# swesterfeld/audiowmark

Hardware: AMD Instinct MI355X
Metric: audio seconds watermarked+decoded per wall-second (xRT), 44.1 kHz stereo (higher is better)
Workload: dtype f32; 1 GPU; 60 min stereo 44.1 kHz white noise per GPU resident in HBM, add+get incl. payload decode, payload 0123456789abcdef0011223344556677, strength 10; parallelism=1 GPU, patterns=108, payload_matches=104, ranks_seen=1

## Files before the change

### audiowmark_amd/binding.py

```python
import ctypes as C
import os

import numpy as np

_HERE = os.path.dirname(os.path.abspath(__file__))
N_BANDS = 81
BLOCK_FRAMES = 2226
SOFT_BITS = 858


class AwmError(RuntimeError):
    pass


def library_path():
    return os.path.join(_HERE, "libawm_hip.so")




def _load_hip_runtime():
    candidates = []
    try:
        import torch
# ... 114 lines not shown
lib.awm_add_watermark_batch_keys_d.argtypes = [_vp, _vp, C.c_char_p, C.c_size_t, _vp, _vp, _vp, C.c_int]
lib.awm_get_watermark_batch_keys_d.argtypes = [_vp, _vp, C.c_size_t, _vp, _vp, C.c_int, C.c_int, C.c_size_t, _vp, _vp]
lib.awm_decode_chunk_d.argtypes = [_vp, _vp, _vp, C.c_size_t, C.c_int, C.c_int, C.c_size_t, _vp]
lib.awm_tab_up_down.argtypes = [_vp, C.c_int, C.c_int, _vp, _vp]
lib.awm_tab_bit_pos.argtypes = [_vp, _vp]
lib.awm_tab_mix_entries.argtypes = [_vp, _vp]
lib.awm_tab_bit_order.argtypes = [_vp, C.c_size_t, _vp]
lib.awm_tab_frame_mod.argtypes = [_vp, C.c_char_p, _vp]
lib.awm_tab_frame_mod_template.argtypes = [_vp, _vp]
lib.awm_tab_sync_bits.argtypes = [_vp, C.c_int, _vp]
lib.awm_tab_window.argtypes = [C.c_size_t, _vp]
lib.awm_tab_synth_window.argtypes = [_vp]
lib.awm_conv_encode.argtypes = [C.c_int, _vp, C.c_size_t, _vp]
lib.awm_test_gen_noise.argtypes = [_vp, C.c_size_t, _vp]


class RawFormat(C.Structure):
    _fields_ = [("n_channels", C.c_int), ("sample_rate", C.c_int), ("bit_depth", C.c_int), ("encoding", C.c_int), ("big_endian", C.c_int)]


lib.awm_add_watermark_file.argtypes = [_vp, _vp, C.c_char_p, C.c_char_p, C.c_char_p, C.POINTER(RawFormat), C.POINTER(RawFormat)]
lib.awm_add_stream_watermark_file.argtypes = [_vp, _vp, C.c_char_p, C.c_char_p, C.c_char_p, C.POINTER(RawFormat), C.POINTER(RawFormat), C.c_size_t]
lib.awm_add_stream_create_at.argtypes = [_vp, _vp, C.c_char_p, C.c_int, C.c_size_t, C.c_size_t, C.POINTER(_vp)]
lib.awm_debug_sync_db_sliding_d.argtypes = [_vp, _vp, C.c_size_t, C.c_int, _vp, C.c_size_t, C.c_int, C.c_int, _vp]
lib.awm_debug_sync_db_sliding_rows_d.argtypes = [_vp, _vp, C.c_size_t, C.c_int, _vp, _vp, C.c_size_t, C.c_int, C.c_int, _vp, _vp, C.c_longlong, C.c_longlong,
                                                 _vp, _vp, C.c_int, C.c_int, C.c_int, _vp, _vp, C.c_longlong, _vp, C.c_longlong]
lib.awm_get_watermark_file.argtypes = [_vp, _vp, C.c_char_p, C.POINTER(RawFormat), C.c_size_t, _vp]
lib.awm_add_get_watermark_file.argtypes = [_vp, _vp, C.c_char_p, C.c_char_p, C.c_char_p, C.POINTER(RawFormat), C.POINTER(RawFormat), C.c_size_t, _vp]
lib.awm_add_stream_create.argtypes = [_vp, _vp, C.c_char_p, C.c_int, C.c_size_t, C.POINTER(_vp)]
lib.awm_add_stream_destroy.argtypes = [_vp]
lib.awm_add_stream_destroy.restype = None
lib.awm_add_stream_input.argtypes = [_vp]
lib.awm_add_stream_input.restype = C.c_void_p
lib.awm_add_stream_push.argtypes = [_vp, C.c_size_t, C.c_int, _vp, _vp]
lib.awm_add_mix_payloads_d.argtypes = [_vp, _vp, _vp, C.c_size_t, C.c_size_t, C.c_int, _vp, C.c_double, C.c_size_t, _vp, _vp, _vp,
                                       C.c_size_t, C.c_size_t]
lib.awm_add_stream_create_payloads_at.argtypes = [_vp, _vp, _vp, C.c_size_t, C.c_int, C.c_size_t, C.c_size_t, C.POINTER(_vp)]
lib.awm_add_stream_payloads.argtypes = [_vp]
lib.awm_add_stream_payloads.restype = C.c_size_t
lib.awm_add_stream_push_payloads.argtypes = [_vp, C.c_size_t, C.c_int, _vp, _vp]
lib.awm_add_watermark_payloads_file.argtypes = [_vp, _vp, _vp, C.c_size_t, C.c_char_p, _vp, C.POINTER(RawFormat), C.POINTER(RawFormat)]
lib.awm_add_stream_watermark_payloads_file.argtypes = [_vp, _vp, _vp, C.c_size_t, C.c_char_p, _vp, C.POINTER(RawFormat), C.POINTER(RawFormat),
                                                       C.c_size_t]
lib.awm_debug_set_payloads_file_tile.argtypes = [C.c_int]
lib.awm_debug_set_payloads_file_tile.restype = None

# ... 520 lines not shown

    def add_watermark_payloads_file(self, key, payloads, in_path, out_paths, raw_in=None, raw_out=None, zero_frames=None):
        payloads = list(payloads)
        outs = check_payload_paths(payloads, in_path, out_paths)
        hexes = (C.c_char_p * len(payloads))(*[p.encode() for p in payloads])
        paths = (C.c_char_p * len(payloads))(*outs)
        rin = C.byref(raw_in) if raw_in is not None else None
        rout = C.byref(raw_out) if raw_out is not None else None
        if zero_frames is not None:
            _check(lib.awm_add_stream_watermark_payloads_file(self._h, key_bytes(key), hexes, len(payloads), os.fsencode(in_path), paths, rin, rout,
                                                              zero_frames), "awm_add_stream_watermark_payloads_file")
            return
        _check(lib.awm_add_watermark_payloads_file(self._h, key_bytes(key), hexes, len(payloads), os.fsencode(in_path), paths, rin, rout),
               "awm_add_watermark_payloads_file")

    def add_get_watermark_file(self, key, payload_hex, in_path, out_path, raw_in=None, raw_out=None):
        return self._patterns(lib.awm_add_get_watermark_file, "awm_add_get_watermark_file", self._h, key_bytes(key), payload_hex.encode(),
                              os.fsencode(in_path), os.fsencode(out_path), C.byref(raw_in) if raw_in is not None else None,
                              C.byref(raw_out) if raw_out is not None else None)

    def get_watermark_file(self, key, in_path, raw_in=None):
        return self._patterns(lib.awm_get_watermark_file, "awm_get_watermark_file", self._h, key_bytes(key), os.fsencode(in_path),
                              C.byref(raw_in) if raw_in is not None else None)

    def sync_db_sliding(self, pcm, bases, count, ld=72):
        import torch
        n, ch = _pcm_shape(pcm)
        b = torch.as_tensor(bases, dtype=torch.int64, device=pcm.device).contiguous()
        out = torch.zeros((b.numel(), 81, ld), dtype=torch.float32, device=pcm.device)
        _check(lib.awm_debug_sync_db_sliding_d(self._h, _dev_ptr(pcm), n, ch, C.c_void_p(b.data_ptr()), b.numel(), count, ld, _dev_ptr(out)),
               "awm_debug_sync_db_sliding_d")
        self.synchronize()
        return out

    def sync_db_sliding_rows(self, pcm, n_frames, bases, counts, count0, rows_per_plane, row_perm, band_pos, first, last, out, have,
                             tail=None, stream_range=None, range_index=None, range_div=1, tables_per_slice=0):
        import torch
        n, ch = _pcm_shape(pcm)
        assert 0 <= n_frames <= n
        want = ((bases, torch.int64, 1), (counts, torch.int32, 1), (row_perm, torch.int32, 0), (band_pos, torch.uint8, 0), (out, torch.float32, 3),
                (have, torch.int8, 2), (tail, torch.float32, 2), (stream_range, torch.int64, 2), (range_index, torch.int32, 1))
        for t, dtype, dim in want:
            assert t is None or (t.dtype == dtype and t.is_cuda and t.is_contiguous() and (not dim or t.dim() == dim))
        assert bases.numel() == counts.numel() and out.shape[1] == 60 and out.shape[0] == have.shape[0] and (tail is None or tail.shape[0] == out.shape[0])
        opt = lambda t: _dev_ptr(t) if t is not None else None
        _check(lib.awm_debug_sync_db_sliding_rows_d(self._h, _dev_ptr(pcm), n_frames, ch, _dev_ptr(bases), _dev_ptr(counts), bases.numel(), count0,
# ... 358 lines not shown
```

### audiowmark_amd/csrc/hip/kernels.hh

```
#pragma once
#include <hip/hip_runtime.h>
#include <cstddef>
#include <cstdint>

#if defined(__HIP_DEVICE_COMPILE__) && !defined(__gfx950__)
#error "audiowmark_amd's HIP kernels are written for gfx950 (MI355X) only"
#endif

namespace awmk {

struct DevTables
{
  const float2 *tw512;
  const float2 *tw1024;
  const float  *window;
  const float  *synth;
  const double2 *slide;
  const double2 *tw512d;
  const float2 *slide32;
};

hipError_t launch_stft_full (hipStream_t st, const DevTables& t, const float *pcm, int n_channels,
                             long long start_index, long long hop, long long frame_count, float2 *out);

struct AddMixArgs
{
  const float *pcm_in;
  float       *out;
  long long    n_frames;
  int          n_channels;
  const int8_t *frame_mod;
  float        neg_delta_up;
  float        neg_delta_down;
  long long    first_frame;
  const float *halo_before;
  const float *halo_after;
  unsigned int *block_max;
  long long    first_block;
  long long    n_blocks;
  int          limiter_block;
  int          frames_per_span;
  int          block_frames = 2226;
  int          frames_pad_start = 250;
// ... 361 lines not shown
```

### audiowmark_amd/csrc/hip/kernels.hip

```cpp
#include "kernels.hh"
#include "awm_fft.hip.h"
#include <cstdlib>
#include <algorithm>
#include <type_traits>

namespace awmk {

constexpr int NB = 81;
constexpr int MIN_BAND = 20;
constexpr int WAVES = 4;

typedef const int __attribute__ ((address_space (4))) *const_int_ptr;

__device__ __forceinline__ void
load_shared_tables (const DevTables& t, float2 *s_tw, float *s_win, float2 *s_twb)
{
  fft512_load_twiddles (t.tw512, s_tw);
  for (int i = threadIdx.x; i < 1024; i += blockDim.x)
    s_win[i] = t.window[i];
  if (s_twb)
    for (int i = threadIdx.x; i < NB; i += blockDim.x)
      s_twb[i] = t.tw1024[MIN_BAND + i];
}

// ... 51 lines not shown
        }
    }
  else
    {
#pragma unroll
      for (int j = 0; j < 8; j++)
        {
          const int x = 2 * (lane + 64 * j);
          v[2 * j]     = x < avail     ? p[(long long) x * C]       : 0.f;
          v[2 * j + 1] = x + 1 < avail ? p[(long long) (x + 1) * C] : 0.f;
        }
    }
}

__device__ __forceinline__ void
window_pack (const float (&v)[16], const float *s_win, int lane, float2 (&z)[8])
{
  const float2 *w2 = reinterpret_cast<const float2 *> (s_win);
#pragma unroll
  for (int j = 0; j < 8; j++)
    {
      const float2 w = lds_ld (&w2[lane + 64 * j]);
      z[j] = make_float2 (__fmul_rn (v[2 * j], w.x), __fmul_rn (v[2 * j + 1], w.y));
    }
}

__global__ void __launch_bounds__ (64 * WAVES)
stft_full_kernel (DevTables t, const float *pcm, int C, long long start_index, long long hop, long long frame_count, float2 *out)
{
  __shared__ float2 s_tw[512];
  __shared__ float  s_win[1024];
  __shared__ float2 s_x[WAVES][XBUF_ELEMS];
  load_shared_tables (t, s_tw, s_win, nullptr);
  __syncthreads();

  const int lane = threadIdx.x & 63, wave = threadIdx.x >> 6;
  const long long item = (long long) blockIdx.x * WAVES + wave;
  if (item >= frame_count * C)
    return;
  const long long f = item / C;
  const int ch = int (item % C);
  float2 *xbuf = s_x[wave];

  float v[16];
  fetch_channel (pcm, start_index + f * hop, 1024, C, ch, lane, v);
  float2 z[8];
// ... 469 lines not shown

  for (long long m = s - 1; m <= e; m++)
    {
      if (OPAQUE)
        {
          lane = lane0;
          asm volatile ("" : "+v" (lane));
        }
      int avail;
      const float *src = frame_source<true> (a.pcm_in, a.n_frames, C, F, m, a.halo_before, a.halo_after, avail);
      float in[CV][16];
      float2 d[CV][8];
      if (avail > 0)
        {
          if constexpr (CV == 2)
            fetch_stereo (src, 0, avail, lane, in[0], in[1]);
          else
            fetch_channel (src, 0, avail, C, ch0, lane, in[0]);
          const long long g = a.first_frame + m;
          const long long row = (frame_number0 + g) % total_rows;
          const int8_t *mod_row = a.frame_mod + row * NB;
          if constexpr (CV == 2 && PAIR)
            {
              window_pack (in[0], s_win, lane, d[0]);
              window_pack (in[1], s_win, lane, d[1]);
              frame_delta2 (d[0], d[1], mod_row, a.neg_delta_up, a.neg_delta_down, xbuf, zd, s_tw, s_tw3, s_twb, lane);
            }
          else
            {
#pragma unroll
              for (int c = 0; c < CV; c++)
                {
                  window_pack (in[c], s_win, lane, d[c]);
                  frame_delta (d[c], mod_row, a.neg_delta_up, a.neg_delta_down, xbuf, zd, s_tw, s_tw3, s_twb, lane);
                }
            }
        }
      else
        {
#pragma unroll
          for (int c = 0; c < CV; c++)
            {
#pragma unroll
              for (int j = 0; j < 16; j++)
                in[c][j] = 0.f;
#pragma unroll
              for (int j = 0; j < 8; j++)
                d[c][j] = make_float2 (0.f, 0.f);
// ... 138 lines not shown
          if constexpr (CV == 2)
            fetch_stereo (src, 0, avail, lane, in[0], in[1]);
          else
            fetch_channel (src, 0, avail, C, ch0, lane, in[0]);
          long long row = (frame_number0 + m) % total_rows;
          if constexpr (SPAN)
            row = (frame_number0 + sp.first_frame + m) % total_rows;
#pragma unroll
          for (int pass = 0; pass < 2; pass++)
            {
              const int k = MIN_BAND + lane + 64 * pass;
              mod[pass] = 0;
#pragma unroll
              for (int p = 0; p < PT; p++)
                if (p < a.n_out && k <= 100)
                  {
                    const int v = a.o[p].frame_mod[row * NB + (k - MIN_BAND)];
                    mod[pass] |= (v ? (v == 1 ? 3 : 1) : 0) << (2 * p);
                  }
            }
          const float e_up = __int_as_float (__builtin_amdgcn_readfirstlane (__float_as_int (0.5f * a.neg_delta_up)));
          const float e_down = __int_as_float (__builtin_amdgcn_readfirstlane (__float_as_int (0.5f * a.neg_delta_down)));
          float2 z[CV][8];
#pragma unroll
          for (int c = 0; c < CV; c++)
            window_pack (in[c], s_win, lane, z[c]);
          if constexpr (CV == 2)
            frame_forward2 (z[0], z[1], xbuf, s_tw, lane);
          else
            frame_forward (z[0], xbuf, s_tw, lane);
#pragma unroll
          for (int pass = 0; pass < 2; pass++)
            {
              const int k = MIN_BAND + lane + 64 * pass;
#pragma unroll
              for (int c = 0; c < CV; c++)
                d_up[c][pass] = d_down[c][pass] = zero;
              if (k <= 100)
                {
                  const float2 w = s_twb[k - MIN_BAND];
#pragma unroll
                  for (int c = 0; c < CV; c++)
                    {
                      float2 X;
                      if (CV == 2 && c == 1)
                        X = real_split (lds_ld (&xbuf[zposb (k)]), lds_ld (&xbuf[zposb (512 - k)]), w);
                      else if (CV == 2)
                        X = real_split (lds_ld (&xbuf[zpos (k)]), lds_ld (&xbuf[zpos (512 - k)]), w);
                      else
                        X = real_split (xbuf[zpos (k)], xbuf[zpos (512 - k)], w);
                      const float abs2 = X.x * X.x + X.y * X.y;
                      if (abs2 > 1e-14f)
                        {
// ... 861 lines not shown
  if (n_channels < 1 || seg.pre < 0 || seg.first_sample < seg.pre || (long long) limiter_block * n_channels < MIX_RUN)
    return hipErrorInvalidValue;
  hipLaunchKernelGGL (mix_max_segment_kernel, dim3 (unsigned ((n_values + MIX_RUN - 1) / MIX_RUN)), dim3 (256), 0, st, seg, n_channels, limiter_block);
  return hipGetLastError();
}

__global__ void
fill_u32_kernel (unsigned int *p, unsigned int v, size_t n)
{
  const size_t i = (size_t) blockIdx.x * blockDim.x + threadIdx.x;
  if (i < n)
    p[i] = v;
}
hipError_t
launch_fill_u32 (hipStream_t st, unsigned int *p, unsigned int v, size_t n)
{
  if (!n)
    return hipSuccess;
  hipLaunchKernelGGL (fill_u32_kernel, dim3 (unsigned ((n + 255) / 256)), dim3 (256), 0, st, p, v, n);
  return hipGetLastError();
}


__device__ __forceinline__ long long
sync_stream_base (const SyncDbArgs& a, long long stream)
{
  if (a.stream_base)
    return a.stream_base[stream];
  if (a.streams_per_slice > 0)
    return a.base0 + (stream % a.streams_per_slice) * a.base_stride + (stream / a.streams_per_slice) * a.slice_stride;
  return a.base0 + stream * a.base_stride;
}

__device__ __forceinline__ void
sync_stream_range (const SyncDbArgs& a, long long stream, long long& first, long long& last)
{
  first = a.first;
  last = a.last;
  if (a.stream_range)
    {
      const long long g = stream / a.range_div;
      const long long slice = a.range_index ? a.range_index[g] : g;
      first = a.stream_range[2 * slice];
      last = a.stream_range[2 * slice + 1];
      if (first < 0)
        first = last = 0x7fffffffffffffffLL;
    }
}


template<int CV, bool SPLIT, int TLD> __global__ void __launch_bounds__ (64 * WAVES)
sync_db_kernel (DevTables t, SyncDbArgs a)
{
  constexpr int TILE_LD = TLD, TILE_MAX = TLD - 1, SPLIT_COLS = TILE_MAX / 2;
  __shared__ float2 s_tw[512];
  __shared__ float  s_win[1024];
  __shared__ float2 s_twb[NB];
  __shared__ float2 s_x[WAVES][XBUF_ELEMS];
  __shared__ float  s_tile[NB * TILE_LD];
  __shared__ char   s_have[TILE_MAX];
  const int lane = threadIdx.x & 63, wave = threadIdx.x >> 6;
  if (a.silent_frames_are_zero && a.skip_unread_silent_tiles)
    {
      long long stream = blockIdx.y, tile_idx = blockIdx.x;
      if (a.xcd_interleave)
        {
          const long long j = blockIdx.x >> 3;
          stream = j % a.n_streams;
          tile_idx = (j / a.n_streams) * 8 + (blockIdx.x & 7);
        }
      const long long base = sync_stream_base (a, stream);
      const int count = a.stream_count ? a.stream_count[stream] : a.count0;
      long long sil_first, sil_last;
      sync_stream_range (a, stream, sil_first, sil_last);
      const long long tile0 = tile_idx * a.tile_frames;
      if (tile0 >= count)
        return;
      const long long n_here = (count - tile0) < a.tile_frames ? count - tile0 : a.tile_frames;
      const long long idx_before = base + (tile0 - 2) * a.hop, idx_after = base + (tile0 + n_here + 1) * a.hop;
      const int C = a.n_channels;
      if ((idx_after + 1024) * C < sil_first || idx_before * C > sil_last)
        return;
    }
  load_shared_tables (t, s_tw, s_win, s_twb);
  __syncthreads();

  long long stream = blockIdx.y, tile_idx = blockIdx.x;
  if (a.xcd_interleave)
    {
      const long long j = blockIdx.x >> 3;
      stream = j % a.n_streams;
      tile_idx = (j / a.n_streams) * 8 + (blockIdx.x & 7);
    }
  const int plane_ch = blockIdx.z;
  const long long base = sync_stream_base (a, stream);
  const int count = a.stream_count ? a.stream_count[stream] : a.count0;
  long long sil_first, sil_last;
  sync_stream_range (a, stream, sil_first, sil_last);
  const int TF = a.tile_frames;
  const long long tile0 = tile_idx * TF;
  if (tile0 >= count)
    return;
  const int C = a.n_channels;
  float2 *xbuf = s_x[wave];
  const int n_here = (count - tile0) < TF ? int (count - tile0) : TF;

  for (int ff = wave; ff < n_here; ff += WAVES)
    {
      const long long idx = base + (tile0 + ff) * a.hop;
      const long long f_first = idx * C, f_last = (idx + 1024) * C;
      const bool outside = idx < 0 || idx + 1024 > a.n_frames;
      const bool skip = (f_last < sil_first) || (f_first > sil_last) || outside;
      float acc0 = 0.f, acc1 = 0.f;
      float split0 = 0.f, split1 = 0.f;
      if (!skip)
        {
          if (CV == 2)
            {
              float in[2][16];
              fetch_stereo (a.pcm, idx, 1024, lane, in[0], in[1]);
              float2 za[8], zb[8];
              window_pack (in[0], s_win, lane, za);
              window_pack (in[1], s_win, lane, zb);
              fft512_forward2 (za, zb, xbuf, s_tw, lane);
              const int k0 = MIN_BAND + lane, k1 = MIN_BAND + 64 + lane;
              const bool second = lane < NB - 64;
              float2 pa[4], pb[4];
              lds_st (&xbuf[0 * 64 + lane], za[0]);
              lds_st (&xbuf[1 * 64 + lane], za[1]);
              lds_st (&xbuf[6 * 64 + lane], za[6]);
              lds_st (&xbuf[7 * 64 + lane], za[7]);
              wave_sync();
              pa[0] = lds_ld (&xbuf[zpos (k0)]);
              pa[1] = lds_ld (&xbuf[zpos (512 - k0)]);
              pa[2] = lds_ld (&xbuf[zpos (second ? k1 : k0)]);
              pa[3] = lds_ld (&xbuf[zpos (512 - (second ? k1 : k0))]);
              wave_sync();
              lds_st (&xbuf[0 * 64 + lane], zb[0]);
              lds_st (&xbuf[1 * 64 + lane], zb[1]);
              lds_st (&xbuf[6 * 64 + lane], zb[6]);
              lds_st (&xbuf[7 * 64 + lane], zb[7]);
              wave_sync();
              pb[0] = lds_ld (&xbuf[zpos (k0)]);
              pb[1] = lds_ld (&xbuf[zpos (512 - k0)]);
              pb[2] = lds_ld (&xbuf[zpos (second ? k1 : k0)]);
              pb[3] = lds_ld (&xbuf[zpos (512 - (second ? k1 : k0))]);
              wave_sync();
              const float2 w0 = s_twb[lane], w1 = s_twb[second ? 64 + lane : lane];
              acc0 = __fadd_rn (acc0, db_from_complex (real_split (pa[0], pa[1], w0)));
              if (second)
                acc1 = __fadd_rn (acc1, db_from_complex (real_split (pa[2], pa[3], w1)));
              if (SPLIT)
                {
                  split0 = acc0;
                  split1 = acc1;
                  acc0 = acc1 = 0.f;
                }
              acc0 = __fadd_rn (acc0, db_from_complex (real_split (pb[0], pb[1], w0)));
              if (second)
                acc1 = __fadd_rn (acc1, db_from_complex (real_split (pb[2], pb[3], w1)));
            }
          else
            {
              const int c_begin = a.per_channel ? plane_ch : 0, c_end = a.per_channel ? plane_ch + 1 : C;
              for (int c = c_begin; c < c_end; c++)
                {
                  float in[16];
                  fetch_channel (a.pcm, idx, 1024, C, c, lane, in);
                  float2 z[8];
// ... 60 lines not shown
          float *out = a.out + stream * a.out_stream_stride + (long long) p * NB * a.ld + tile0;
          for (int i = threadIdx.x; i < NB * n_here; i += blockDim.x)
            {
              const int band = i / n_here, ff = i - band * n_here;
              out[band * a.ld + ff] = s_tile[band * TILE_LD + p * SPLIT_COLS + ff];
            }
        }
    }
  else
    {
      const long long plane = a.per_channel ? plane_ch : 0;
      float *out = a.out + stream * a.out_stream_stride + plane * NB * a.ld + tile0;
      for (int i = threadIdx.x; i < NB * n_here; i += blockDim.x)
        {
          const int band = i / n_here, ff = i - band * n_here;
          out[band * a.ld + ff] = s_tile[band * TILE_LD + ff];
        }
    }
  if (a.have && plane_ch == 0)
    for (int i = threadIdx.x; i < n_here; i += blockDim.x)
      a.have[stream * a.have_stream_stride + tile0 + i] = s_have[i];
}

hipError_t
launch_sync_db (hipStream_t st, const DevTables& t, const SyncDbArgs& a)
{
  if (a.n_streams <= 0 || a.tile_frames <= 0 || a.tile_frames > 72)
    return a.n_streams <= 0 ? hipSuccess : hipErrorInvalidValue;
  int max_count = a.count0;
  if (max_count <= 0)
    return hipSuccess;
  const unsigned tiles = unsigned ((max_count + a.tile_frames - 1) / a.tile_frames);
  if (a.n_streams > 65535LL * 1)
    {
      SyncDbArgs b = a;
      long long done = 0;
      while (done < a.n_streams)
        {
          const long long n = (a.n_streams - done) > 65535 ? 65535 : (a.n_streams - done);
          b.n_streams = n;
          b.base0 = a.base0 + done * a.base_stride;
          b.stream_base = a.stream_base ? a.stream_base + done : nullptr;
          b.stream_count = a.stream_count ? a.stream_count + done : nullptr;
          b.out = a.out + done * a.out_stream_stride;
          b.have = a.have ? a.have + done * a.have_stream_stride : nullptr;
          hipError_t e = launch_sync_db (st, t, b);
          if (e != hipSuccess)
            return e;
          done += n;
        }
      return hipSuccess;
    }
  const bool small = a.tile_frames <= 32;
  if (a.n_channels == 2 && a.per_channel)
    {
      SyncDbArgs b = a;
      b.tile_frames = 16;
      const unsigned split_tiles = unsigned ((max_count + b.tile_frames - 1) / b.tile_frames);
      hipLaunchKernelGGL ((sync_db_kernel<2, true, 33>), dim3 (split_tiles, unsigned (a.n_streams), 1), dim3 (64 * WAVES), 0, st, t, b);
      return hipGetLastError();
    }
  const unsigned planes = a.per_channel ? unsigned (a.n_channels) : 1u;
  dim3 grid (tiles, unsigned (a.n_streams), planes);
  SyncDbArgs b = a;
  if (!a.stream_base && !a.stream_count && a.n_streams >= 2 && a.n_streams <= 8 && planes == 1)
    {
      b.xcd_interleave = 1;
      grid = dim3 (unsigned (((tiles + 7) / 8) * 8 * a.n_streams), 1, 1);
    }
  if (a.n_channels == 2 && !a.per_channel)
    {
      if (small)
        hipLaunchKernelGGL ((sync_db_kernel<2, false, 33>), grid, dim3 (64 * WAVES), 0, st, t, b);
      else
        hipLaunchKernelGGL ((sync_db_kernel<2, false, 73>), grid, dim3 (64 * WAVES), 0, st, t, b);
    }
  else
    {
      if (small)
        hipLaunchKernelGGL ((sync_db_kernel<1, false, 33>), grid, dim3 (64 * WAVES), 0, st, t, b);
      else
        hipLaunchKernelGGL ((sync_db_kernel<1, false, 73>), grid, dim3 (64 * WAVES), 0, st, t, b);
    }
  return hipGetLastError();
}

constexpr int SL_TILE = 16;

__device__ __forceinline__ double
dpp_from_lower_lane (double v)
{
  const int lo = __builtin_amdgcn_update_dpp (0, __double2loint (v), 0x138, 0xf, 0xf, true);
  const int hi = __builtin_amdgcn_update_dpp (0, __double2hiint (v), 0x138, 0xf, 0xf, true);
  return __hiloint2double (hi, lo);
}
// ... 1966 lines not shown
```

### audiowmark_amd/csrc/host/capi_kernels.cc

```cpp
#include "context.hh"
#include "syncfinder.hh"
#include "wmget.hh"
#include "wmspeed.hh"
#include "utils.hh"
#include "wmfile.hh"
#include <sys/stat.h>
#include <atomic>
#include <future>
#include <thread>
#include <tuple>
#include <algorithm>
#include <cmath>
#include <cstdlib>
#include <cstring>
#include <memory>

using namespace awm;
namespace awm { Key capi_key (const uint8_t key[16]); }
namespace awm { extern int g_key_tables_on_device; int clip_key_tables_check (awm_ctx *ctx, const uint8_t *keys, size_t n_keys, long long mismatch_out[9]); }

namespace {

constexpr int LIMITER_BLOCK = Params::mark_sample_rate * int (Params::limiter_block_size_ms) / 1000;
const float LIMITER_CEILING = float (Params::limiter_ceiling);
// ... 899 lines not shown
      const int zero = 0;
      AWM_HIP_CHECK (hipMemcpyAsync (ctx->ws_misc.ptr, &zero, sizeof (int), hipMemcpyHostToDevice, ctx->stream));
      AWM_HIP_CHECK (hipMemcpyAsync (ctx->ws_misc.as<char>() + sizeof (int), pos.data(), pos.size(), hipMemcpyHostToDevice, ctx->stream));
      da.row_perm = ctx->ws_misc.as<int>();
      da.band_pos = ctx->ws_misc.as<unsigned char>() + sizeof (int);
      da.rows_per_plane = 1;
      da.out_stream_stride = 60 * 64;
      if (awmk::sliding_rows_have_tail (n_channels))
        {
          da.tail = out_d + n_streams * 60 * 64;
          da.tail_stream_stride = 60;
        }
      else if (count > 64)
        {
          set_error ("awm_debug_sync_db_sliding_d: rows of 64 offsets take 65 only with forms 4 / 5");
          return AWM_ERR_ARG;
        }
    }
  AWM_HIP_CHECK (awmk::launch_sync_db_sliding (ctx->stream, ctx->tabs, da));
  return 0;
}

int
awm_debug_sync_db_sliding_rows_d (awm_ctx *ctx, const float *pcm_d, size_t n_frames, int n_channels, const long long *base_d, const int *count_d,
                                  size_t n_streams, int count0, int rows_per_plane, const int *row_perm_d, const unsigned char *band_pos_d,
                                  long long first, long long last, const long long *stream_range_d, const int *range_index_d, int range_div,
                                  int tables_per_slice, int ld, float *out_d, float *tail_d, long long tail_stream_stride, char *have_d,
                                  long long have_stream_stride)
{
  AWM_ENTER (ctx);
  const char *bad = nullptr;
  if (!pcm_d || !base_d || !count_d || !row_perm_d || !band_pos_d || !out_d || !have_d)
    bad = "null pointer";
  else if (n_channels != 1 && n_channels != 2)
    bad = "1 or 2 channels";
  else if (count0 < 0 || count0 > 65 || have_stream_stride < count0)
    bad = "count0 within 0 .. 65 and within a stream's have flags";
  else if (rows_per_plane < 1 || range_div < 1 || (tables_per_slice != 0 && tables_per_slice != 1))
    bad = "rows_per_plane, range_div or tables_per_slice";
  else if (tail_d && (!awmk::sliding_rows_have_tail (n_channels) || tail_stream_stride < 60))
    bad = "only forms 4 / 5 write a tail (stereo), 60 values per stream";
  else if (ld < std::min (count0, tail_d ? 64 : 65))
    bad = "ld below the offsets of a row (64 only with a tail)";
  if (!bad && n_streams)
    {
      std::vector<long long> base (n_streams);
// ... 2352 lines not shown
```

### audiowmark_amd/csrc/host/context.cc

```cpp
#include "context.hh"
#include <algorithm>
#include <atomic>
#include <chrono>
#include <cstdlib>
#include "utils.hh"
#include <cmath>
#include <cstring>

namespace awm {

static thread_local std::string g_last_error;
void set_error (const std::string& msg) { g_last_error = msg; }
const std::string& last_error() { return g_last_error; }
std::string hip_error_string (hipError_t e) { return std::string (hipGetErrorName (e)) + " (" + hipGetErrorString (e) + ")"; }

static std::atomic<long>   g_dev_allocs { 0 }, g_pin_allocs { 0 };
static std::atomic<double> g_dev_alloc_ms { 0.0 }, g_pin_alloc_ms { 0.0 };
static std::atomic<unsigned long long> g_dev_alloc_bytes { 0 };
static void
note_alloc (std::atomic<long>& count, std::atomic<double>& ms, std::chrono::steady_clock::time_point t0)
{
  const double dt = std::chrono::duration<double, std::milli> (std::chrono::steady_clock::now() - t0).count();
  count.fetch_add (1, std::memory_order_relaxed);
  double cur = ms.load (std::memory_order_relaxed);
// ... 650 lines not shown
  auto ctx = std::make_unique<awm_ctx>();
  ctx->device = device;
  if (own_stream)
    AWM_HIP_CHECK (hipStreamCreateWithFlags (&ctx->stream, hipStreamNonBlocking));
  else
    ctx->stream = given;
  ctx->own_stream = own_stream;

  std::vector<float> blob;
  auto push_c = [&] (double re, double im) { blob.push_back (float (re)); blob.push_back (float (im)); };
  const size_t off_tw512 = blob.size();
  for (int k = 0; k < 512; k++)
    push_c (std::cos (-2 * M_PI * k / 512), std::sin (-2 * M_PI * k / 512));
  const size_t off_tw1024 = blob.size();
  for (int k = 0; k <= 512; k++)
    push_c (std::cos (-2 * M_PI * k / 1024), std::sin (-2 * M_PI * k / 1024));
  while (blob.size() % 4) blob.push_back (0);
  const size_t off_win = blob.size();
  auto win = gen_normalized_window (Params::frame_size);
  blob.insert (blob.end(), win.begin(), win.end());
  const size_t off_synth = blob.size();
  auto synth = gen_synth_window();
  blob.insert (blob.end(), synth.begin(), synth.end());
  std::vector<double> slide;
  for (int k = 19; k <= 102; k++)
    {
      for (int j = 0; j < 8; j++)
        {
          slide.push_back (std::cos (-2 * M_PI * k * j / 1024));
          slide.push_back (std::sin (-2 * M_PI * k * j / 1024));
        }
      slide.push_back (std::cos (2 * M_PI * k * 8 / 1024));
      slide.push_back (std::sin (2 * M_PI * k * 8 / 1024));
    }
  const size_t off_tw512d = slide.size();
  for (int k = 0; k < 512; k++)
    {
      slide.push_back (std::cos (-2 * M_PI * k / 512));
      slide.push_back (std::sin (-2 * M_PI * k / 512));
    }
  const size_t off_slide32 = slide.size();
  {
    std::vector<float> f;
    for (int k = 19; k <= 102; k++)
      for (int j = 0; j < 8; j++)
        {
          f.push_back (float (std::cos (2 * M_PI * k * (8 - j) / 1024)));
          f.push_back (float (std::sin (2 * M_PI * k * (8 - j) / 1024)));
        }
    slide.resize (off_slide32 + f.size() / 2);
    std::memcpy (slide.data() + off_slide32, f.data(), f.size() * sizeof (float));
  }
  if (int rc = upload (ctx->tab_slide, slide.data(), slide.size() * sizeof (double), ctx->stream))
    return rc;
  ctx->tabs.slide = ctx->tab_slide.as<double2>();
  ctx->tabs.tw512d = reinterpret_cast<const double2 *> (ctx->tab_slide.as<double>() + off_tw512d);
  ctx->tabs.slide32 = reinterpret_cast<const float2 *> (ctx->tab_slide.as<double>() + off_slide32);
  if (int rc = upload (ctx->tab_mem, blob.data(), blob.size() * sizeof (float), ctx->stream))
    return rc;
  const float *base = ctx->tab_mem.as<float>();
  ctx->tabs.tw512 = reinterpret_cast<const float2 *> (base + off_tw512);
  ctx->tabs.tw1024 = reinterpret_cast<const float2 *> (base + off_tw1024);
  ctx->tabs.window = base + off_win;
  ctx->tabs.synth = base + off_synth;
  if (awmk::probe_dependent_launch_us (ctx->stream) < 0 && hipStreamSynchronize (ctx->stream) != hipSuccess)
    {
      set_error ("awm_ctx_create: the device does not complete work on the context's stream");
      return AWM_ERR_HIP;
    }
  *ctx_out = ctx.release();
  return 0;
}

int
awm_ctx_set_chunk_lanes (awm_ctx *ctx, int n_lanes)
{
  if (!ctx || n_lanes < 1)
    return AWM_ERR_ARG;
  ctx->chunk_lanes = std::min (n_lanes, awm::CHUNK_LANES);
  return 0;
}

int
awm_ctx_warm_up (awm_ctx *ctx, int detect_speed, int file_level)
{
  if (!ctx)
    return AWM_ERR_ARG;
// ... 132 lines not shown
```

### include/awm_hip.h

```cpp
#ifndef AWM_HIP_H
#define AWM_HIP_H

#include <stddef.h>
#include <stdint.h>

#ifdef __cplusplus
extern "C" {
#endif

#define AWM_ERR_GENERIC    (-1)
#define AWM_ERR_NO_DEVICE  (-2)
#define AWM_ERR_ARG        (-3)
#define AWM_ERR_HIP        (-4)
#define AWM_ERR_IO         (-5)

#define AWM_FRAME_SIZE      1024
#define AWM_N_BANDS         81
#define AWM_BLOCK_FRAMES    2226
#define AWM_SOFT_BITS       858

typedef struct awm_ctx awm_ctx;

const char *awm_last_error (void);
const char *awm_version (void);
// ... 208 lines not shown
int awm_speed_clip_location_d (awm_ctx *ctx, const uint8_t key[16], const float *pcm_d, size_t n_frames, int n_channels, int rate,
                               double seconds, int candidates, double *location);
int awm_speed_mags_d (awm_ctx *ctx, const uint8_t key[16], const float *pcm_d, size_t n_frames, int n_channels, int rate,
                      double clip_location, double center, double seconds, size_t max_rows, float *out);
int awm_speed_scan_d (awm_ctx *ctx, const uint8_t key[16], const float *pcm_d, size_t n_frames, int n_channels, int rate,
                      double clip_location, double seconds, double step, int n_steps, int n_center_steps,
                      const double *speeds, int n_speeds, size_t max_out, double *out_speed, double *out_quality);

int    awm_speed_select_n_best (double *speed, double *quality, int count, int n);
double awm_speed_smooth_best (const double *speed, const double *quality, int count, double step, double distance);
size_t awm_speed_clip_positions (const uint8_t key[16], size_t n_values, size_t max_out, uint64_t *positions);
int    awm_speed_clip_candidates (const uint8_t key[16], const float *hashed_values, size_t n, int candidates, double *locations);

void awm_debug_set_viterbi_super (int on);
void awm_debug_set_viterbi_persistent (int on);
double awm_debug_dependent_launch_us (void);
int  awm_debug_viterbi_one_launch_in_use (void);
void awm_debug_set_sliding3 (int on);
void awm_debug_set_refine_form (int form);
int  awm_debug_refine_form (void);
void awm_debug_set_k4s_ablate (int flags);
int  awm_debug_sync_db_sliding_d (awm_ctx *ctx, const float *pcm_d, size_t n_frames, int n_channels, const long long *base_d, size_t n_streams,
                                  int count, int ld, float *out_d);
int  awm_debug_sync_db_sliding_rows_d (awm_ctx *ctx, const float *pcm_d, size_t n_frames, int n_channels, const long long *base_d, const int *count_d,
                                       size_t n_streams, int count0, int rows_per_plane, const int *row_perm_d, const unsigned char *band_pos_d,
                                       long long first, long long last, const long long *stream_range_d, const int *range_index_d, int range_div,
                                       int tables_per_slice, int ld, float *out_d, float *tail_d, long long tail_stream_stride, char *have_d,
                                       long long have_stream_stride);
void awm_debug_set_soft_bits_generic (int on);
void awm_debug_set_scan_generic (int on);
int  awm_debug_scan_generic_launches (void);
void awm_debug_set_chunk_stagger (int mode);
void awm_debug_set_resample_phase (int on);
void awm_debug_set_get_overlap (int on);
void awm_debug_set_speed_compare_wide (int on);
void awm_debug_set_speed_compare_fold (int on);
void awm_debug_set_resample_var_mode (int mode);
void awm_debug_set_speed_overlap (int on);
int  awm_debug_frame_mod_tables_d (awm_ctx *ctx, const uint8_t *keys, size_t n_keys, const char *payload_hex, int8_t *tables_out);
int  awm_debug_clip_key_tables_check_d (awm_ctx *ctx, const uint8_t *keys, size_t n_keys, long long mismatch_out[9]);
void awm_debug_set_key_tables_on_device (int on);
void awm_debug_set_merge_decodes (int on);
void awm_debug_set_add_batched (int on);
void awm_debug_set_add_slab_mb (int mb);
void awm_debug_set_add_payloads_fused (int on);
int  awm_debug_add_payloads_fused_in_use (void);
// ... 52 lines not shown
```

Before: 756,200 xRT.

## Fuse stereo window packing and add optional resident sync_db kernel

Adds window_pack2, which windows both stereo channels in one loop with a single window load per element, and uses it in the add and sync_db paths. The sync_db stereo path now reads band bins for both channels straight from the two-channel forward FFT buffer (zposb) instead of storing each channel's outputs back to LDS and reloading them, which drops several LDS stores and wave syncs. It also adds a persistent 'resident' sync_db kernel that loops over tiles and loads a prepacked table image once per workgroup, but this path is off by default behind a debug switch. Adds a debug entry point and Python binding for sync_db.

```diff
diff --git a/audiowmark_amd/binding.py b/audiowmark_amd/binding.py
--- a/audiowmark_amd/binding.py
+++ b/audiowmark_amd/binding.py
@@ -160,6 +160,12 @@
 lib.awm_add_watermark_file.argtypes = [_vp, _vp, C.c_char_p, C.c_char_p, C.c_char_p, C.POINTER(RawFormat), C.POINTER(RawFormat)]
 lib.awm_add_stream_watermark_file.argtypes = [_vp, _vp, C.c_char_p, C.c_char_p, C.c_char_p, C.POINTER(RawFormat), C.POINTER(RawFormat), C.c_size_t]
 lib.awm_add_stream_create_at.argtypes = [_vp, _vp, C.c_char_p, C.c_int, C.c_size_t, C.c_size_t, C.POINTER(_vp)]
+lib.awm_debug_sync_db_d.argtypes = [_vp, _vp, C.c_size_t, C.c_int, C.c_int, C.c_longlong, C.c_longlong, _vp, C.c_size_t, C.c_int, C.c_int, C.c_longlong,
+                                    C.c_longlong, C.c_longlong, C.c_int, _vp, _vp]
+lib.awm_debug_set_sync_db_resident.argtypes = [C.c_int]
+lib.awm_debug_set_sync_db_resident.restype = None
+lib.awm_debug_set_sync_db_max_workgroups.argtypes = [C.c_int]
+lib.awm_debug_set_sync_db_max_workgroups.restype = None
 lib.awm_debug_sync_db_sliding_d.argtypes = [_vp, _vp, C.c_size_t, C.c_int, _vp, C.c_size_t, C.c_int, C.c_int, _vp]
 lib.awm_debug_sync_db_sliding_rows_d.argtypes = [_vp, _vp, C.c_size_t, C.c_int, _vp, _vp, C.c_size_t, C.c_int, C.c_int, _vp, _vp, C.c_longlong, C.c_longlong,
                                                  _vp, _vp, C.c_int, C.c_int, C.c_int, _vp, _vp, C.c_longlong, _vp, C.c_longlong]
@@ -726,6 +732,18 @@
     def get_watermark_file(self, key, in_path, raw_in=None):
         return self._patterns(lib.awm_get_watermark_file, "awm_get_watermark_file", self._h, key_bytes(key), os.fsencode(in_path),
                               C.byref(raw_in) if raw_in is not None else None)
+
+    def sync_db(self, pcm, count, out, n_streams=1, base0=0, base_stride=0, bases=None, per_channel=False, tile_frames=32, first=0, last=None,
+                flags=0, have=None):
+        n, ch = _pcm_shape(pcm)
+        if last is None:
+            last = n * ch
+        planes = ch if per_channel else 1
+        assert out.is_contiguous() and out.numel() == n_streams * planes * N_BANDS * out.shape[-1]
+        assert have is None or (have.is_contiguous() and have.numel() == n_streams * out.shape[-1])
+        _check(lib.awm_debug_sync_db_d(self._h, _dev_ptr(pcm), n, ch, int(per_channel), base0, base_stride, _dev_ptr(bases) if bases is not None else None,
+                                       n_streams, count, tile_frames, out.shape[-1], first, last, flags, _dev_ptr(out),
+                                       _dev_ptr(have) if have is not None else None), "awm_debug_sync_db_d")
 
     def sync_db_sliding(self, pcm, bases, count, ld=72):
         import torch
diff --git a/audiowmark_amd/csrc/hip/kernels.hh b/audiowmark_amd/csrc/hip/kernels.hh
--- a/audiowmark_amd/csrc/hip/kernels.hh
+++ b/audiowmark_amd/csrc/hip/kernels.hh
@@ -18,7 +18,16 @@
   const double2 *slide;
   const double2 *tw512d;
   const float2 *slide32;
-};
+  const float4 *sync_db_image;
+};
+
+constexpr int
+fft512_twiddle_index (int i)
+{
+  return i < 448 ? (i & 63) * ((i >> 6) + 1) : 8 * ((i - 448) & 7) * (((i - 448) >> 3) + 1);
+}
+constexpr int SYNC_DB_IMAGE_TW = 0, SYNC_DB_IMAGE_WIN = 1024, SYNC_DB_IMAGE_TWB = 2048, SYNC_DB_IMAGE_FLOATS = 2212;
+static_assert (SYNC_DB_IMAGE_FLOATS % 4 == 0 && SYNC_DB_IMAGE_FLOATS >= SYNC_DB_IMAGE_TWB + 2 * 81, "whole float4 pieces");
 
 hipError_t launch_stft_full (hipStream_t st, const DevTables& t, const float *pcm, int n_channels,
                              long long start_index, long long hop, long long frame_count, float2 *out);
diff --git a/audiowmark_amd/csrc/hip/kernels.hip b/audiowmark_amd/csrc/hip/kernels.hip
--- a/audiowmark_amd/csrc/hip/kernels.hip
+++ b/audiowmark_amd/csrc/hip/kernels.hip
@@ -1,5 +1,6 @@
 #include "kernels.hh"
 #include "awm_fft.hip.h"
+#include <cstddef>
 #include <cstdlib>
 #include <algorithm>
 #include <type_traits>
@@ -97,6 +98,19 @@
     {
       const float2 w = lds_ld (&w2[lane + 64 * j]);
       z[j] = make_float2 (__fmul_rn (v[2 * j], w.x), __fmul_rn (v[2 * j + 1], w.y));
+    }
+}
+
+__device__ __forceinline__ void
+window_pack2 (const float (&va)[16], const float (&vb)[16], const float *s_win, int lane, float2 (&za)[8], float2 (&zb)[8])
+{
+  const float2 *w2 = reinterpret_cast<const float2 *> (s_win);
+#pragma unroll
+  for (int j = 0; j < 8; j++)
+    {
+      const float2 w = lds_ld (&w2[lane + 64 * j]);
+      za[j] = make_float2 (__fmul_rn (va[2 * j], w.x), __fmul_rn (va[2 * j + 1], w.y));
+      zb[j] = make_float2 (__fmul_rn (vb[2 * j], w.x), __fmul_rn (vb[2 * j + 1], w.y));
     }
 }
 
@@ -612,8 +626,7 @@
           const int8_t *mod_row = a.frame_mod + row * NB;
           if constexpr (CV == 2 && PAIR)
             {
-              window_pack (in[0], s_win, lane, d[0]);
-              window_pack (in[1], s_win, lane, d[1]);
+              window_pack2 (in[0], in[1], s_win, lane, d[0], d[1]);
               frame_delta2 (d[0], d[1], mod_row, a.neg_delta_up, a.neg_delta_down, xbuf, zd, s_tw, s_tw3, s_twb, lane);
             }
           else
@@ -798,13 +811,16 @@
           const float e_up = __int_as_float (__builtin_amdgcn_readfirstlane (__float_as_int (0.5f * a.neg_delta_up)));
           const float e_down = __int_as_float (__builtin_amdgcn_readfirstlane (__float_as_int (0.5f * a.neg_delta_down)));
           float2 z[CV][8];
-#pragma unroll
-          for (int c = 0; c < CV; c++)
-            window_pack (in[c], s_win, lane, z[c]);
           if constexpr (CV == 2)
-            frame_forward2 (z[0], z[1], xbuf, s_tw, lane);
+            {
+              window_pack2 (in[0], in[1], s_win, lane, z[0], z[1]);
+              frame_forward2 (z[0], z[1], xbuf, s_tw, lane);
+            }
           else
-            frame_forward (z[0], xbuf, s_tw, lane);
+            {
+              window_pack (in[0], s_win, lane, z[0]);
+              frame_forward (z[0], xbuf, s_tw, lane);
+            }
 #pragma unroll
           for (int pass = 0; pass < 2; pass++)
             {
@@ -1712,8 +1728,8 @@
 }
 
 
-__device__ __forceinline__ long long
-sync_stream_base (const SyncDbArgs& a, long long stream)
+template<class ARGS> __device__ __forceinline__ long long
+sync_stream_base (const ARGS& a, long long stream)
 {
   if (a.stream_base)
     return a.stream_base[stream];
@@ -1722,8 +1738,8 @@
   return a.base0 + stream * a.base_stride;
 }
 
-__device__ __forceinline__ void
-sync_stream_range (const SyncDbArgs& a, long long stream, long long& first, long long& last)
+template<class ARGS> __device__ __forceinline__ void
+sync_stream_range (const ARGS& a, long long stream, long long& first, long long& last)
 {
   first = a.first;
   last = a.last;
@@ -1739,50 +1755,44 @@
 }
 
 
-template<int CV, bool SPLIT, int TLD> __global__ void __launch_bounds__ (64 * WAVES)
-sync_db_kernel (DevTables t, SyncDbArgs a)
+template<class ARGS> __device__ __forceinline__ bool
+sync_db_tile_unread (const ARGS& a, long long stream, long long tile_idx)
+{
+  const long long base = sync_stream_base (a, stream);
+  const int count = a.stream_count ? a.stream_count[stream] : a.count0;
+  long long sil_first, sil_last;
+  sync_stream_range (a, stream, sil_first, sil_last);
+  const long long tile0 = tile_idx * a.tile_frames;
+  if (tile0 >= count)
+    return true;
+  const long long n_here = (count - tile0) < a.tile_frames ? count - tile0 : a.tile_frames;
+  const long long idx_before = base + (tile0 - 2) * a.hop, idx_after = base + (tile0 + n_here + 1) * a.hop;
+  const int C = a.n_channels;
+  return (idx_after + 1024) * C < sil_first || idx_before * C > sil_last;
+}
+
+template<class ARGS> __device__ __forceinline__ void
+sync_db_item (const ARGS& a, long long id, unsigned tiles_x, long long& stream, long long& tile_idx)
+{
+  if (a.xcd_interleave)
+    {
+      const long long j = id >> 3;
+      stream = j % a.n_streams;
+      tile_idx = (j / a.n_streams) * 8 + (id & 7);
+    }
+  else
+    {
+      stream = id / tiles_x;
+      tile_idx = id - stream * tiles_x;
+    }
+}
+
+template<int CV, bool SPLIT, int TLD, class ARGS> __device__ __forceinline__ void
+sync_db_tile (const ARGS& a, long long stream, long long tile_idx, int plane_ch, const float2 *s_tw, const float *s_win, const float2 *s_twb,
+              float2 *s_x, float *s_tile, char *s_have)
 {
   constexpr int TILE_LD = TLD, TILE_MAX = TLD - 1, SPLIT_COLS = TILE_MAX / 2;
-  __shared__ float2 s_tw[512];
-  __shared__ float  s_win[1024];
-  __shared__ float2 s_twb[NB];
-  __shared__ float2 s_x[WAVES][XBUF_ELEMS];
-  __shared__ float  s_tile[NB * TILE_LD];
-  __shared__ char   s_have[TILE_MAX];
   const int lane = threadIdx.x & 63, wave = threadIdx.x >> 6;
-  if (a.silent_frames_are_zero && a.skip_unread_silent_tiles)
-    {
-      long long stream = blockIdx.y, tile_idx = blockIdx.x;
-      if (a.xcd_interleave)
-        {
-          const long long j = blockIdx.x >> 3;
-          stream = j % a.n_streams;
-          tile_idx = (j / a.n_streams) * 8 + (blockIdx.x & 7);
-        }
-      const long long base = sync_stream_base (a, stream);
-      const int count = a.stream_count ? a.stream_count[stream] : a.count0;
-      long long sil_first, sil_last;
-      sync_stream_range (a, stream, sil_first, sil_last);
-      const long long tile0 = tile_idx * a.tile_frames;
-      if (tile0 >= count)
-        return;
-      const long long n_here = (count - tile0) < a.tile_frames ? count - tile0 : a.tile_frames;
-      const long long idx_before = base + (tile0 - 2) * a.hop, idx_after = base + (tile0 + n_here + 1) * a.hop;
-      const int C = a.n_channels;
-      if ((idx_after + 1024) * C < sil_first || idx_before * C > sil_last)
-        return;
-    }
-  load_shared_tables (t, s_tw, s_win, s_twb);
-  __syncthreads();
-
-  long long stream = blockIdx.y, tile_idx = blockIdx.x;
-  if (a.xcd_interleave)
-    {
-      const long long j = blockIdx.x >> 3;
-      stream = j % a.n_streams;
-      tile_idx = (j / a.n_streams) * 8 + (blockIdx.x & 7);
-    }
-  const int plane_ch = blockIdx.z;
   const long long base = sync_stream_base (a, stream);
   const int count = a.stream_count ? a.stream_count[stream] : a.count0;
   long long sil_first, sil_last;
@@ -1792,7 +1802,7 @@
   if (tile0 >= count)
     return;
   const int C = a.n_channels;
-  float2 *xbuf = s_x[wave];
+  float2 *xbuf = s_x + wave * XBUF_ELEMS;
   const int n_here = (count - tile0) < TF ? int (count - tile0) : TF;
 
   for (int ff = wave; ff < n_here; ff += WAVES)
@@ -1810,31 +1820,19 @@
               float in[2][16];
               fetch_stereo (a.pcm, idx, 1024, lane, in[0], in[1]);
               float2 za[8], zb[8];
-              window_pack (in[0], s_win, lane, za);
-              window_pack (in[1], s_win, lane, zb);
-              fft512_forward2 (za, zb, xbuf, s_tw, lane);
+              window_pack2 (in[0], in[1], s_win, lane, za, zb);
+              frame_forward2 (za, zb, xbuf, s_tw, lane);
               const int k0 = MIN_BAND + lane, k1 = MIN_BAND + 64 + lane;
               const bool second = lane < NB - 64;
               float2 pa[4], pb[4];
-              lds_st (&xbuf[0 * 64 + lane], za[0]);
-              lds_st (&xbuf[1 * 64 + lane], za[1]);
-              lds_st (&xbuf[6 * 64 + lane], za[6]);
-              lds_st (&xbuf[7 * 64 + lane], za[7]);
-              wave_sync();
               pa[0] = lds_ld (&xbuf[zpos (k0)]);
               pa[1] = lds_ld (&xbuf[zpos (512 - k0)]);
               pa[2] = lds_ld (&xbuf[zpos (second ? k1 : k0)]);
               pa[3] = lds_ld (&xbuf[zpos (512 - (second ? k1 : k0))]);
-              wave_sync();
-              lds_st (&xbuf[0 * 64 + lane], zb[0]);
-              lds_st (&xbuf[1 * 64 + lane], zb[1]);
-              lds_st (&xbuf[6 * 64 + lane], zb[6]);
-              lds_st (&xbuf[7 * 64 + lane], zb[7]);
-              wave_sync();
-              pb[0] = lds_ld (&xbuf[zpos (k0)]);
-              pb[1] = lds_ld (&xbuf[zpos (512 - k0)]);
-              pb[2] = lds_ld (&xbuf[zpos (second ? k1 : k0)]);
-              pb[3] = lds_ld (&xbuf[zpos (512 - (second ? k1 : k0))]);
+              pb[0] = lds_ld (&xbuf[zposb (k0)]);
+              pb[1] = lds_ld (&xbuf[zposb (512 - k0)]);
+              pb[2] = lds_ld (&xbuf[zposb (second ? k1 : k0)]);
+              pb[3] = lds_ld (&xbuf[zposb (512 - (second ? k1 : k0))]);
               wave_sync();
               const float2 w0 = s_twb[lane], w1 = s_twb[second ? 64 + lane : lane];
               acc0 = __fadd_rn (acc0, db_from_complex (real_split (pa[0], pa[1], w0)));
@@ -1941,6 +1939,95 @@
       a.have[stream * a.have_stream_stride + tile0 + i] = s_have[i];
 }
 
+template<int CV, bool SPLIT, int TLD> __global__ void __launch_bounds__ (64 * WAVES)
+sync_db_kernel (DevTables t, SyncDbArgs a)
+{
+  __shared__ float2 s_tw[512];
+  __shared__ float  s_win[1024];
+  __shared__ float2 s_twb[NB];
+  __shared__ float2 s_x[WAVES][XBUF_ELEMS];
+  __shared__ float  s_tile[NB * TLD];
+  __shared__ char   s_have[TLD - 1];
+  long long stream = blockIdx.y, tile_idx = blockIdx.x;
+  if (a.xcd_interleave)
+    sync_db_item (a, blockIdx.x, 0, stream, tile_idx);
+  if (a.silent_frames_are_zero && a.skip_unread_silent_tiles && sync_db_tile_unread (a, stream, tile_idx))
+    return;
+  load_shared_tables (t, s_tw, s_win, s_twb);
+  __syncthreads();
+  sync_db_tile<CV, SPLIT, TLD> (a, stream, tile_idx, blockIdx.z , s_tw, s_win, s_twb, &s_x[0][0], s_tile, s_have);
+}
+
+struct SyncDbResidentParams
+{
+  DevTables    t;
+  SyncDbArgs   a;
+  unsigned int n_items, tiles_x;
+};
+template<int CV, bool SPLIT, int TLD> __global__ void __launch_bounds__ (64 * WAVES)
+sync_db_resident_kernel (SyncDbResidentParams p)
+{
+  __shared__ float4 s_tab[SYNC_DB_IMAGE_FLOATS / 4];
+  __shared__ float2 s_x[WAVES][XBUF_ELEMS];
+  __shared__ float  s_tile[NB * TLD];
+  __shared__ char   s_have[TLD - 1];
+  for (int i = threadIdx.x; i < SYNC_DB_IMAGE_FLOATS / 4; i += blockDim.x)
+    s_tab[i] = p.t.sync_db_image[i];
+  __syncthreads();
+  const float *s_f = reinterpret_cast<const float *> (s_tab);
+  const float2 *s_tw = reinterpret_cast<const float2 *> (s_f + SYNC_DB_IMAGE_TW), *s_twb = reinterpret_cast<const float2 *> (s_f + SYNC_DB_IMAGE_TWB);
+  const float *s_win = s_f + SYNC_DB_IMAGE_WIN;
+  const unsigned n_items = p.n_items, tiles_x = p.tiles_x;
+  for (unsigned id = blockIdx.x; id < n_items; id += gridDim.x)
+    {
+      typedef const SyncDbArgs __attribute__ ((address_space (4))) *const_args_ptr;
+      typedef const char __attribute__ ((address_space (4))) *const_char_ptr;
+      const_args_ptr ap = (const_args_ptr) ((const_char_ptr) __builtin_amdgcn_kernarg_segment_ptr() + offsetof (SyncDbResidentParams, a));
+      asm volatile ("" : "+s" (ap));
+      long long stream, tile_idx;
+      sync_db_item (*ap, id, tiles_x, stream, tile_idx);
+      if (ap->silent_frames_are_zero && ap->skip_unread_silent_tiles && sync_db_tile_unread (*ap, stream, tile_idx))
+        continue;
+      sync_db_tile<CV, SPLIT, TLD> (*ap, stream, tile_idx, 0, s_tw, s_win, s_twb, &s_x[0][0], s_tile, s_have);
+      __syncthreads();
+    }
+}
+
+constexpr int SYNC_DB_RESIDENT_DEFAULT = 0;
+static int g_sync_db_resident = SYNC_DB_RESIDENT_DEFAULT, g_sync_db_max_workgroups = 0;
+extern "C" void awm_debug_set_sync_db_resident (int mode) { g_sync_db_resident = (mode >= 0 && mode <= 2) ? mode : SYNC_DB_RESIDENT_DEFAULT; }
+extern "C" void awm_debug_set_sync_db_max_workgroups (int n) { g_sync_db_max_workgroups = n > 0 ? n : 0; }
+
+static unsigned
+sync_db_resident_slots()
+{
+  static int slots[64];
+  int dev = 0;
+  if (hipGetDevice (&dev) != hipSuccess || dev < 0 || dev >= 64)
+    return 1024;
+  if (!slots[dev])
+    {
+      int cus = 0;
+      if (hipDeviceGetAttribute (&cus, hipDeviceAttributeMultiprocessorCount, dev) != hipSuccess || cus <= 0)
+        return 1024;
+      slots[dev] = 4 * cus;
+    }
+  return unsigned (slots[dev]);
+}
+
+static unsigned
+sync_db_resident_grid (unsigned long long n_items, bool interleave, bool split)
+{
+  if (!g_sync_db_resident || (g_sync_db_resident == 2 && !split) || n_items >= (1ULL << 31))
+    return 0;
+  unsigned long long g = std::min<unsigned long long> (n_items, sync_db_resident_slots());
+  if (g_sync_db_max_workgroups)
+    g = std::min<unsigned long long> (g, g_sync_db_max_workgroups);
+  if (interleave && g >= 8)
+    g &= ~7ULL;
+  return unsigned (g);
+}
+
 hipError_t
 launch_sync_db (hipStream_t st, const DevTables& t, const SyncDbArgs& a)
 {
@@ -1976,7 +2063,11 @@
       SyncDbArgs b = a;
       b.tile_frames = 16;
       const unsigned split_tiles = unsigned ((max_count + b.tile_frames - 1) / b.tile_frames);
-      hipLaunchKernelGGL ((sync_db_kernel<2, true, 33>), dim3 (split_tiles, unsigned (a.n_streams), 1), dim3 (64 * WAVES), 0, st, t, b);
+      const unsigned long long n_items = (unsigned long long) split_tiles * a.n_streams;
+      if (const unsigned resident = sync_db_resident_grid (n_items, false, true))
+        hipLaunchKernelGGL ((sync_db_resident_kernel<2, true, 33>), dim3 (resident), dim3 (64 * WAVES), 0, st, SyncDbResidentParams { t, b, unsigned (n_items), split_tiles });
+      else
+        hipLaunchKernelGGL ((sync_db_kernel<2, true, 33>), dim3 (split_tiles, unsigned (a.n_streams), 1), dim3 (64 * WAVES), 0, st, t, b);
       return hipGetLastError();
     }
   const unsigned planes = a.per_channel ? unsigned (a.n_channels) : 1u;
@@ -1989,7 +2080,11 @@
     }
   if (a.n_channels == 2 && !a.per_channel)
     {
-      if (small)
+      const unsigned long long n_items = (unsigned long long) grid.x * grid.y;
+      const unsigned resident = small ? sync_db_resident_grid (n_items, b.xcd_interleave, false) : 0;
+      if (resident)
+        hipLaunchKernelGGL ((sync_db_resident_kernel<2, false, 33>), dim3 (resident), dim3 (64 * WAVES), 0, st, SyncDbResidentParams { t, b, unsigned (n_items), grid.x });
+      else if (small)
         hipLaunchKernelGGL ((sync_db_kernel<2, false, 33>), grid, dim3 (64 * WAVES), 0, st, t, b);
       else
         hipLaunchKernelGGL ((sync_db_kernel<2, false, 73>), grid, dim3 (64 * WAVES), 0, st, t, b);
diff --git a/audiowmark_amd/csrc/host/capi_kernels.cc b/audiowmark_amd/csrc/host/capi_kernels.cc
--- a/audiowmark_amd/csrc/host/capi_kernels.cc
+++ b/audiowmark_amd/csrc/host/capi_kernels.cc
@@ -945,6 +945,43 @@
 }
 
 int
+awm_debug_sync_db_d (awm_ctx *ctx, const float *pcm_d, size_t n_frames, int n_channels, int per_channel, long long base0, long long base_stride,
+                     const long long *base_d, size_t n_streams, int count, int tile_frames, long long ld, long long first, long long last, int flags,
+                     float *out_d, char *have_d)
+{
+  AWM_ENTER (ctx);
+  if (!pcm_d || !out_d || count < 1 || ld < count || tile_frames < 1 || tile_frames > 72 || (n_channels != 1 && n_channels != 2) || !n_streams ||
+      (flags & ~3) || ((flags & 2) && !(flags & 1)))
+    {
+      set_error ("awm_debug_sync_db_d: bad argument");
+      return AWM_ERR_ARG;
+    }
+  awmk::SyncDbArgs da {};
+  da.pcm = pcm_d;
+  da.n_frames = (long long) n_frames;
+  da.n_channels = n_channels;
+  da.per_channel = per_channel ? 1 : 0;
+  da.base0 = base0;
+  da.base_stride = base_stride;
+  da.stream_base = base_d;
+  da.count0 = count;
+  da.n_streams = (long long) n_streams;
+  da.hop = Params::frame_size;
+  da.out = out_d;
+  da.out_stream_stride = (long long) (per_channel ? n_channels : 1) * Params::n_bands * ld;
+  da.ld = ld;
+  da.have = have_d;
+  da.have_stream_stride = ld;
+  da.first = first;
+  da.last = last;
+  da.silent_frames_are_zero = flags & 1;
+  da.skip_unread_silent_tiles = (flags >> 1) & 1;
+  da.tile_frames = tile_frames;
+  AWM_HIP_CHECK (awmk::launch_sync_db (ctx->stream, ctx->tabs, da));
+  return 0;
+}
+
+int
 awm_debug_sync_db_sliding_rows_d (awm_ctx *ctx, const float *pcm_d, size_t n_frames, int n_channels, const long long *base_d, const int *count_d,
                                   size_t n_streams, int count0, int rows_per_plane, const int *row_perm_d, const unsigned char *band_pos_d,
                                   long long first, long long last, const long long *stream_range_d, const int *range_index_d, int range_div,
diff --git a/audiowmark_amd/csrc/host/context.cc b/audiowmark_amd/csrc/host/context.cc
--- a/audiowmark_amd/csrc/host/context.cc
+++ b/audiowmark_amd/csrc/host/context.cc
@@ -696,6 +696,16 @@
   const size_t off_synth = blob.size();
   auto synth = gen_synth_window();
   blob.insert (blob.end(), synth.begin(), synth.end());
+  while (blob.size() % 4) blob.push_back (0);
+  const size_t off_image = blob.size();
+  blob.resize (off_image + awmk::SYNC_DB_IMAGE_FLOATS, 0.f);
+  for (int i = 0; i < 504; i++)
+    for (int c = 0; c < 2; c++)
+      blob[off_image + awmk::SYNC_DB_IMAGE_TW + 2 * i + c] = blob[off_tw512 + 2 * awmk::fft512_twiddle_index (i) + c];
+  for (size_t i = 0; i < Params::frame_size; i++)
+    blob[off_image + awmk::SYNC_DB_IMAGE_WIN + i] = blob[off_win + i];
+  for (int i = 0; i < 2 * Params::n_bands; i++)
+    blob[off_image + awmk::SYNC_DB_IMAGE_TWB + i] = blob[off_tw1024 + 2 * Params::min_band + i];
   std::vector<double> slide;
   for (int k = 19; k <= 102; k++)
     {
@@ -737,6 +747,7 @@
   ctx->tabs.tw1024 = reinterpret_cast<const float2 *> (base + off_tw1024);
   ctx->tabs.window = base + off_win;
   ctx->tabs.synth = base + off_synth;
+  ctx->tabs.sync_db_image = reinterpret_cast<const float4 *> (base + off_image);
   if (awmk::probe_dependent_launch_us (ctx->stream) < 0 && hipStreamSynchronize (ctx->stream) != hipSuccess)
     {
       set_error ("awm_ctx_create: the device does not complete work on the context's stream");
diff --git a/include/awm_hip.h b/include/awm_hip.h
--- a/include/awm_hip.h
+++ b/include/awm_hip.h
@@ -254,6 +254,11 @@
 void awm_debug_set_k4s_ablate (int flags);
 int  awm_debug_sync_db_sliding_d (awm_ctx *ctx, const float *pcm_d, size_t n_frames, int n_channels, const long long *base_d, size_t n_streams,
                                   int count, int ld, float *out_d);
+int  awm_debug_sync_db_d (awm_ctx *ctx, const float *pcm_d, size_t n_frames, int n_channels, int per_channel, long long base0, long long base_stride,
+                          const long long *base_d, size_t n_streams, int count, int tile_frames, long long ld, long long first, long long last, int flags,
+                          float *out_d, char *have_d);
+void awm_debug_set_sync_db_resident (int mode);
+void awm_debug_set_sync_db_max_workgroups (int n);
 int  awm_debug_sync_db_sliding_rows_d (awm_ctx *ctx, const float *pcm_d, size_t n_frames, int n_channels, const long long *base_d, const int *count_d,
                                        size_t n_streams, int count0, int rows_per_plane, const int *row_perm_d, const unsigned char *band_pos_d,
                                        long long first, long long last, const long long *stream_range_d, const int *range_index_d, int range_div,
```

Result: no change. 757,700 xRT, median of 4 (+0.2%).
